# zhangmozhe/Deep-Exemplar-based-Video-Colorization

Measured on AMD Instinct MI355X. Metric: colorized frames/sec/GPU at 216x384; correlation HBM GB/s vs roofline, higher is better.
Workload: dtype f32

## Files before the change

deep-exemplar-based-video-colorization_amd/csrc/conv_mfma.hip:

```cpp
#include "conv_kernel.h"
#include "conv_sk_kernel.h"
#include <algorithm>

#include "conv_wino_kernel.h"

static int virt_dim(int S, int up, int sub) {
    if (up == 2) return S * 2;
    if (sub == 2) return (S + 1) / 2;
    return S;
}

extern "C" int dvc_conv2d_out_hw(const DvcConvDesc* d, int32_t* OH, int32_t* OW) {
    DVC_REQUIRE(d, "dvc_conv2d_out_hw: null descriptor");
    int VH = virt_dim(d->H, d->in_up, d->in_sub), VW = virt_dim(d->W, d->in_up, d->in_sub);
    int ext = d->dil * (d->ksize - 1) + 1;
    *OH = (VH + 2 * d->pad - ext) / d->stride + 1;
    *OW = (VW + 2 * d->pad - ext) / d->stride + 1;
    return 0;
}

static int pick_tw(int OW) {
    int best = 32, best_w = cdiv(OW, 32) * 32;
    for (int tw : {16, 8}) {
        int wpad = cdiv(OW, tw) * tw;
// ... 484 lines not shown
    int m, tr, S;
    wino_plan(d, OH, OW, workspace_bytes > 0, workspace_bytes, &m, &tr, &S);
    DVC_REQUIRE(m >= 0, "dvc_conv2d_winograd_split: no configuration for cfg %d / split_k %d on this layer", d->cfg, d->split_k);
    const int kc = kWinoShapes[m].kc, nch = d->Cin / kc;
    *split = cdiv(nch, cdiv(nch, S));
    *images_per_launch = wino_images_per_launch(d, OH, OW, m, tr, *split, workspace_bytes);
    return 0;
}

static int wino_setup(const DvcConvDesc* d, const DvcConvDesc* d2, const float* x, const float* x2, const float* u_packed,
                      const float* bias, const float* act_slope_ptr, const float* residual, float* y, void* workspace,
                      size_t workspace_bytes, float* pool, long pool_batch_stride, ConvWinoArgs& s, int* m_out, int* tr_out,
                      int* group_out) {
    DVC_REQUIRE(d && x && u_packed && (y || pool), "dvc_conv2d_winograd: null argument");
    DVC_REQUIRE(d->ksize == 3 && d->stride == 1 && (d->dil == 1 || d->dil == 2) && d->pad == d->dil,
                "dvc_conv2d_winograd: needs a 3x3 stride-1 layer with pad == dilation (1 or 2)");
    DVC_REQUIRE(!d->in_prelu, "dvc_conv2d_winograd: no fused input transform on this path");
    DVC_REQUIRE((d->in_up == 1 || d->in_up == 2) && (d->in_sub == 1 || d->in_sub == 2) && !(d->in_up == 2 && d->in_sub == 2),
                "dvc_conv2d_winograd: bad in_up/in_sub");
    DVC_REQUIRE(d->N > 0 && d->Cin > 0 && d->H > 0 && d->W > 0 && d->Cout > 0, "dvc_conv2d_winograd: bad shape");
    DVC_REQUIRE(d->Cin % 8 == 0 && d->Cout % 64 == 0, "dvc_conv2d_winograd: needs Cin %% 8 == 0 and Cout %% 64 == 0 (got %d, %d)",
                d->Cin, d->Cout);
    DVC_REQUIRE((reinterpret_cast<uintptr_t>(u_packed) & 15) == 0, "dvc_conv2d_winograd: weights must be 16-byte aligned");
    DVC_REQUIRE((long)d->Cin * d->H * d->W * 4 < (1L << 31) && (long)d->Cin * 2048 * 4 < (1L << 31),
                "dvc_conv2d_winograd: tensor too large for buffer-descriptor staging");
    s.x2 = nullptr; s.x2_bs = 0; s.cinA = d->Cin; s.H2 = s.W2 = s.VH2 = s.VW2 = 0; s.in_up2 = s.in_sub2 = 1;
    ConvKArgs& a = s.k;
    a.x = x; a.w = u_packed; a.bias = bias; a.in_scale = nullptr; a.in_shift = nullptr;
    a.in_slope_ptr = nullptr; a.act_slope_ptr = act_slope_ptr; a.res = residual; a.y = y;
    a.N = d->N; a.Cin = d->Cin; a.H = d->H; a.W = d->W;
    a.VH = virt_dim(d->H, d->in_up, d->in_sub);
    a.VW = virt_dim(d->W, d->in_up, d->in_sub);
    int32_t OH, OW;
    dvc_conv2d_out_hw(d, &OH, &OW);
    DVC_REQUIRE(OH > 0 && OW > 0, "dvc_conv2d_winograd: empty output");
    if (d->pad_mode == DVC_PAD_REFLECT)
        DVC_REQUIRE(d->pad < a.VH && d->pad < a.VW, "dvc_conv2d_winograd: reflect pad needs pad < input size");
    a.Cout = d->Cout; a.OH = OH; a.OW = OW;
    a.ks = 3; a.stride = 1; a.dil = d->dil; a.pad = d->pad; a.pad_mode = d->pad_mode;
    a.in_up = d->in_up; a.in_sub = d->in_sub; a.act = d->act; a.in_prelu = 0;
    a.act_slope = d->act_slope;
    a.x_bs = d->x_batch_stride ? d->x_batch_stride : (long)d->Cin * d->H * d->W;
    a.y_bs = d->y_batch_stride ? d->y_batch_stride : (long)d->Cout * OH * OW;
    a.res_bs = d->res_batch_stride ? d->res_batch_stride : (long)d->Cout * OH * OW;
    a.cin_pad = d->Cin; a.IH_T = a.IW_T = a.IW_P = 0;
    a.dbg = g_conv_dbg; a.dbg_buf = nullptr; a.w_bs = 0; a.gray = 0;
    s.ss = d->dil;
    const int TY = cdiv(cdiv(OH, s.ss), 2), TX = cdiv(cdiv(OW, s.ss), 2);
    int best_m = -1, best_tr = 1, best_S = 1;
    if (d2) {
        s.x2 = x2;
        s.cinA = d->Cin - d2->Cin;
        s.H2 = d2->H; s.W2 = d2->W;
        s.VH2 = virt_dim(d2->H, d2->in_up, d2->in_sub);
        s.VW2 = virt_dim(d2->W, d2->in_up, d2->in_sub);
        s.in_up2 = d2->in_up; s.in_sub2 = d2->in_sub;
        s.x2_bs = d2->x_batch_stride ? d2->x_batch_stride : (long)d2->Cin * d2->H * d2->W;
        DVC_REQUIRE(s.VH2 == a.VH && s.VW2 == a.VW, "dvc_conv2d_winograd_dual: the two inputs' virtual sizes differ (%d x %d vs %d x %d)",
                    a.VH, a.VW, s.VH2, s.VW2);
        DVC_REQUIRE((long)d2->Cin * d2->H * d2->W * 4 < (1L << 31), "dvc_conv2d_winograd_dual: second input too large");
        a.x_bs = d->x_batch_stride ? d->x_batch_stride : (long)s.cinA * d->H * d->W;
    }
    wino_plan(d, OH, OW, workspace != nullptr, workspace_bytes, &best_m, &best_tr, &best_S, d2 ? 2 : -1);
    DVC_REQUIRE(best_m >= 0, "dvc_conv2d_winograd: no configuration for cfg %d / split_k %d on this layer", d->cfg, d->split_k);
    const int wm = kWinoShapes[best_m].wm, wn = kWinoShapes[best_m].wn, kc = kWinoShapes[best_m].kc;
    const int nch = d->Cin / kc;
    s.blk_y = cdiv(TY, best_tr * wn);
    s.blk_x = cdiv(TX, 32 / best_tr);
    a.chunks_per_split = cdiv(nch, best_S);
    a.split = cdiv(nch, a.chunks_per_split);
    a.part = reinterpret_cast<float*>(workspace);
    s.gx = s.ss * s.ss * s.blk_y * s.blk_x;
    s.gy = d->Cout / (32 * wm);
    const int group = wino_images_per_launch(d, OH, OW, best_m, best_tr, a.split, workspace_bytes);
    DVC_REQUIRE(group >= 0, "dvc_conv2d_winograd: %ld workgroups per image (feature map too large for this path)",
                (long)s.gx * s.gy * a.split);
    DVC_REQUIRE(group > 0, "dvc_conv2d_winograd: split-K workspace too small for one image");
    DVC_REQUIRE(!(d->flags & DVC_CONV_DEFER_REDUCE) || a.split == 1 || group >= d->N,
                "dvc_conv2d_winograd: DVC_CONV_DEFER_REDUCE needs a workspace that holds the partial sums of the whole batch");
    DVC_REQUIRE(!(d->flags & DVC_CONV_DEFER_REDUCE) || a.split == 1 || !residual,
                "dvc_conv2d_winograd: DVC_CONV_DEFER_REDUCE does not carry a residual");
    s.pool_bs = pool_batch_stride ? pool_batch_stride : (long)d->Cout * (OH / 2) * (OW / 2);
    s.pool = pool;
    *m_out = best_m; *tr_out = best_tr; *group_out = group;
    return 0;
}

static dim3 wino_finish_grid(ConvWinoArgs& s, int NB) {
    s.gz = NB * s.k.split;
    s.m_gxy = wino_magic((long)s.gx * s.gy);
    s.m_gx = wino_magic(s.gx);
    s.m_cls = wino_magic((long)s.blk_y * s.blk_x);
    s.m_blkx = wino_magic(s.blk_x);
    s.m_split = wino_magic(s.k.split);
    return dim3((unsigned)(s.gx * s.gy * s.gz));
}

static int wino_reduce(const DvcConvDesc* d, const ConvWinoArgs& s, int NB, int OH, int OW, const float* bias,
                       const float* act_slope_ptr, hipStream_t st) {
    const ConvKArgs& a = s.k;
    const long OHW = (long)OH * OW, per_img = (long)d->Cout * OHW;
    if (a.split > 1 && s.pool) {
        const long windows = (long)d->Cout * ((OH + 1) / 2) * ((OW + 1) / 2);
        hipLaunchKernelGGL(conv_splitk_reduce_pool_kernel, dim3((unsigned)((windows + 255) / 256), NB), dim3(256), 0, st, a.part,
                           a.split, (long)NB * per_img, d->Cout, OH, OW, bias, d->act, d->act_slope, act_slope_ptr, a.y, a.y_bs,
                           s.pool, s.pool_bs);
        DVC_CHECK_LAUNCH("dvc_conv2d_winograd_pool(split-K reduce)");
    } else if (a.split > 1 && !(d->flags & DVC_CONV_DEFER_REDUCE)) {
        const bool v4 = (OHW % 4 == 0) && ((reinterpret_cast<uintptr_t>(a.part) & 15) == 0) && (((long)NB * per_img) % 4 == 0);
        if (v4)
            hipLaunchKernelGGL(conv_splitk_reduce_kernel<4>, dim3((unsigned)((per_img / 4 + 255) / 256), NB), dim3(256), 0, st,
                               a.part, a.split, (long)NB * per_img, d->Cout, OHW, bias, a.res, a.res_bs, d->act,
                               d->act_slope, act_slope_ptr, a.y, a.y_bs);
        else
            hipLaunchKernelGGL(conv_splitk_reduce_kernel<1>, dim3((unsigned)((per_img + 255) / 256), NB), dim3(256), 0, st,
                               a.part, a.split, (long)NB * per_img, d->Cout, OHW, bias, a.res, a.res_bs, d->act,
                               d->act_slope, act_slope_ptr, a.y, a.y_bs);
        DVC_CHECK_LAUNCH("dvc_conv2d_winograd(split-K reduce)");
    }
    return 0;
}

static int wino_run(const DvcConvDesc* d, const DvcConvDesc* d2, const float* x, const float* x2, const float* u_packed,
                    const float* bias, const float* act_slope_ptr, const float* residual, float* y, void* workspace,
                    size_t workspace_bytes, dvcStream stream, float* pool = nullptr, long pool_batch_stride = 0) {
    ConvWinoArgs s;
    int best_m = -1, best_tr = 1, group = 0;
    if (int rc = wino_setup(d, d2, x, x2, u_packed, bias, act_slope_ptr, residual, y, workspace, workspace_bytes, pool,
                            pool_batch_stride, s, &best_m, &best_tr, &group))
        return rc;
    ConvKArgs& a = s.k;
    int32_t OH, OW;
    dvc_conv2d_out_hw(d, &OH, &OW);
    hipStream_t st = (hipStream_t)stream;
    for (int n0 = 0; n0 < d->N; n0 += group) {
        const int NB = std::min(group, d->N - n0);
        a.N = NB;
        a.x = x + (long)n0 * a.x_bs;
        if (d2) s.x2 = x2 + (long)n0 * s.x2_bs;
        a.y = y ? y + (long)n0 * a.y_bs : nullptr;
        s.pool = pool ? pool + (long)n0 * s.pool_bs : nullptr;
        a.res = residual ? residual + (long)n0 * a.res_bs : nullptr;
        DVC_REQUIRE((long)s.gx * s.gy * NB * a.split < (1L << 31), "dvc_conv2d_winograd: grid too large");
        const dim3 grid = wino_finish_grid(s, NB);
        if (d2) conv_wino_launch_m1_dual(best_tr, grid, st, s);
        else if (best_m == 0) conv_wino_launch_m4(best_tr, grid, st, s);
        else if (best_m == 1) conv_wino_launch_m2(best_tr, grid, st, s);
        else if (best_m == 2) conv_wino_launch_m1(best_tr, grid, st, s);
        else conv_wino_launch_m0(best_tr, grid, st, s);
        DVC_CHECK_LAUNCH("dvc_conv2d_winograd");
        if (int rc = wino_reduce(d, s, NB, OH, OW, bias, act_slope_ptr, st)) return rc;
    }
    return 0;
}

extern "C" int dvc_conv2d_winograd_group(const DvcConvGroupItem* items, int32_t n_items, dvcStream stream) {
    DVC_REQUIRE(items && n_items >= 1 && n_items <= WINO_GROUP_MAX, "dvc_conv2d_winograd_group: 1..%d items", WINO_GROUP_MAX);
    hipStream_t st = (hipStream_t)stream;
    ConvWinoGroupArgs g;
    int OHs[WINO_GROUP_MAX], OWs[WINO_GROUP_MAX], order[WINO_GROUP_MAX];
    ConvWinoArgs tmp[WINO_GROUP_MAX];
    int trs[WINO_GROUP_MAX];
    bool together = n_items > 1;
    for (int i = 0; i < n_items; ++i) {
        const DvcConvGroupItem& it = items[i];
        DVC_REQUIRE(it.x && it.u_packed && it.y, "dvc_conv2d_winograd_group: null argument in item %d", i);
// ... 127 lines not shown
```

deep-exemplar-based-video-colorization_amd/csrc/conv_wino_kernel.h:

```cpp
#pragma once
#include <type_traits>

#include "conv_kernel.h"

typedef float f32x4 __attribute__((ext_vector_type(4)));
typedef float f32x2 __attribute__((ext_vector_type(2)));

struct ConvWinoArgs {
    ConvKArgs k;
    int ss;
    int blk_y, blk_x;
    int gx, gy, gz;
    unsigned m_gx, m_gxy, m_cls, m_blkx, m_split;
    const float* x2;
    long x2_bs;
    int cinA, H2, W2, VH2, VW2, in_up2, in_sub2;
    float* pool;
    long pool_bs;
};
__host__ __device__ __forceinline__ unsigned wino_magic(long d) {
    return d > 1 ? (unsigned)(((1ULL << 32) + (unsigned long long)d - 1) / (unsigned long long)d) : 0u;
}
__device__ __forceinline__ int wino_div(int n, unsigned magic) { return magic ? (int)__umulhi((unsigned)n, magic) : n; }

__host__ __device__ constexpr int wino_pitch(int tr) { return tr == 1 ? 66 : tr == 2 ? 48 : tr == 4 ? 24 : 12; }

#define WINO_A10(p) "a" #p "0", "a" #p "1", "a" #p "2", "a" #p "3", "a" #p "4", "a" #p "5", "a" #p "6", "a" #p "7", "a" #p "8", "a" #p "9"
#define WINO_AGPRS                                                                                                     \
    WINO_A10(), WINO_A10(1), WINO_A10(2), WINO_A10(3), WINO_A10(4), WINO_A10(5), WINO_A10(6), WINO_A10(7), WINO_A10(8), \
        WINO_A10(9), WINO_A10(10), WINO_A10(11), "a120", "a121", "a122", "a123", "a124", "a125", "a126", "a127"
#define WINO_MFMA(K, A, B)                                                                \
    asm volatile("s_nop 1\n\tv_mfma_f32_32x32x2_f32 a[%2:%3], %0, %1, a[%2:%3]"            \
                 :                                                                         \
                 : "v"(A), "v"(B), "i"((K) * 16), "i"((K) * 16 + 15)                       \
                 : WINO_AGPRS)
#define WINO_PK_ADD(D, A, B) asm volatile("v_pk_add_f32 %0, %1, %2" : "=v"(D) : "v"(A), "v"(B))
#define WINO_PK_SUB(D, A, B) asm volatile("v_pk_add_f32 %0, %1, %2 neg_lo:[0,1] neg_hi:[0,1]" : "=v"(D) : "v"(A), "v"(B))
#define WINO_PK_MID(D, A, B) \
    asm volatile("v_pk_add_f32 %0, %1, %2 op_sel:[0,1] op_sel_hi:[0,1] neg_hi:[0,1]" : "=v"(D) : "v"(A), "v"(B))

#define WINO_LOADS(D, U, XA, UA, UOFS)                                                                                 \
    asm volatile("ds_read2_b64 %0, %5 offset0:%7 offset1:%8\n\t"                                                        \
                 "ds_read2_b64 %1, %5 offset0:%9 offset1:%10\n\t"                                                       \
                 "ds_read2_b64 %2, %5 offset0:%11 offset1:%12\n\t"                                                      \
                 "ds_read_b128 %3, %6 offset:%13\n\t"                                                                   \
                 "ds_read_b128 %4, %6 offset:%14"                                                                       \
                 : "=&v"(D[0]), "=&v"(D[1]), "=&v"(D[2]), "=&v"(U[0]), "=&v"(U[1])                                      \
                 : "v"(XA), "v"(UA), "i"(0 * (PITCH / 2)), "i"(0 * (PITCH / 2) + 1), "i"(1 * (PITCH / 2)),              \
                   "i"(1 * (PITCH / 2) + 1), "i"(2 * (PITCH / 2)), "i"(2 * (PITCH / 2) + 1), "i"((UOFS) + 0),           \
                   "i"((UOFS) + 512)                                                                                    \
                 : "memory")
#define WINO_WAIT_LOADS(D, U)                                                                 \
    asm volatile("s_waitcnt lgkmcnt(0)"                                                        \
                 : "+v"(D[0]), "+v"(D[1]), "+v"(D[2]), "+v"(U[0]), "+v"(U[1])                  \
                 :                                                                             \
                 : "memory")

#define WINO_S_ADD(D, A, B) asm volatile("v_add_f32 %0, %1, %2" : "=v"(D) : "v"(A), "v"(B))
#define WINO_S_SUB(D, A, B) asm volatile("v_sub_f32 %0, %1, %2" : "=v"(D) : "v"(A), "v"(B))

__device__ __forceinline__ int wino_stored_offset(int VH, int VW, int W, int in_up, int in_sub, int pad_mode, int vy, int vx) {
    int sy = map_virtual(vy, VH, pad_mode);
    int sx = map_virtual(vx, VW, pad_mode);
    if (sy < 0 || sx < 0) return -1;
    if (in_up == 2) {
        sy >>= 1;
        sx >>= 1;
    } else if (in_sub == 2) {
        sy <<= 1;
        sx <<= 1;
    }
    return sy * W + sx;
}

#define WINO_NBUF 3
__host__ __device__ constexpr int wino_xs_floats(int wm, int wn, int tr, int kc) {
    return ((kc * (2 * tr * wn + 2) * wino_pitch(tr) + 128 * wm * wn - 1) / (128 * wm * wn)) * (128 * wm * wn);
}
__host__ __device__ constexpr int wino_us_floats(int wm, int kc) { return wm * kc * 128 * 4; }

template <int WM, int WN, int TR, int KC, int VAR = 0, bool DUAL = false, class SA = ConvWinoArgs>
__device__ __forceinline__ void conv_wino_body(const SA& s, const int wlog, float* const xsb, float* const usb) {
#if defined(__HIP_DEVICE_COMPILE__)
    const auto& a = s.k;
    constexpr int NPAIR = WM * WN;
    constexpr int NT = 128 * NPAIR;
    constexpr int TC = 32 / TR;
    constexpr int PR = 2 * TR * WN + 2;
    constexpr int PC = 2 * TC + 2;
    constexpr int PITCH = wino_pitch(TR);
    constexpr int plane = PR * PITCH;
    constexpr int EPT = (KC * plane + NT - 1) / NT;
    constexpr int C_XS = EPT * NT;
    static_assert(C_XS == wino_xs_floats(WM, WN, TR, KC), "LDS size helper out of step");
    constexpr int UQ = WM * KC * 128;
    static_assert(UQ * 4 == wino_us_floats(WM, KC), "LDS size helper out of step");
    static_assert(UQ % NT == 0, "whole staging instructions");
    static_assert(PITCH >= PC && PITCH % 2 == 0 && plane % 2 == 0 && KC % 4 == 0, "aligned patch rows, even K-steps per chunk");
    static_assert(2 * (PITCH / 2) + 1 < 256, "ds_read2_b64 offsets are 8 bits");
    constexpr int WPT = UQ / NT;
    constexpr int NI = EPT + WPT;
    static_assert(2 * NI < 64, "vmcnt is 6 bits");
    constexpr int KS = KC / 2;
    constexpr int NBUF = WINO_NBUF;
    constexpr int OOB = (int)0x80000000;
    static_assert(NBUF * UQ * 4 >= 2 * NPAIR * 32 * 64, "the output exchange fits in the filter buffers");

    const int tid = threadIdx.x;
    const int lane = tid & 63, wave = __builtin_amdgcn_readfirstlane(tid >> 6);
    const int l31 = lane & 31, hi = lane >> 5;
    const int ph = wave / NPAIR, pair = wave % NPAIR;
    const int wm = pair / WN, wn = pair % WN;
    const int tr = l31 / TC, tc = l31 % TC;
    const int ss = s.ss;
    const int bz = wino_div(wlog, s.m_gxy), r_xy = wlog - bz * (s.gx * s.gy);
    const int by = wino_div(r_xy, s.m_gx), bx = r_xy - by * s.gx;
    const int per_cls = s.blk_y * s.blk_x;
    const int cls = wino_div(bx, s.m_cls), brem = bx - cls * per_cls;
    const int py = ss == 2 ? cls >> 1 : 0, px = ss == 2 ? cls & 1 : 0;
    const int tyb = wino_div(brem, s.m_blkx);
    const int ty0 = tyb * (TR * WN), tx0 = (brem - tyb * s.blk_x) * TC;
    const int b0 = by * WM;
    const int n = wino_div(bz, s.m_split), ksplit = bz - n * a.split;
    const int HWi = a.H * a.W;

    const int nchunks_all = a.Cin / KC;
    const int c_begin = ksplit * a.chunks_per_split;
    const int c_end = min(nchunks_all, c_begin + a.chunks_per_split);

    int gofs[EPT], wrel[WPT];
#pragma unroll
    for (int i = 0; i < WPT; ++i) {
        const int q = tid + i * NT;
        wrel[i] = ((q / (KC * 128)) * a.Cin * 128 + q % (KC * 128)) * 16;
    }
    __amdgpu_buffer_rsrc_t rs_w =
        __builtin_amdgcn_make_buffer_rsrc((void*)(a.w + (long)b0 * a.Cin * 512), 0, WM * a.Cin * 2048, 0x00020000);
    auto issue_w = [&](int c, int buf) {
        const int sw = c * KC * 2048;
        float* us = usb + buf * (UQ * 4);
#pragma unroll
        for (int i = 0; i < WPT; ++i)
            __builtin_amdgcn_raw_ptr_buffer_load_lds(rs_w, (CONV_AS3 void*)(us + (i * NT + wave * 64) * 4), 16, wrel[i], sw, 0, 0);
    };
    issue_w(c_begin, 0);
    asm volatile(".set wino_i, 0\n\t.rept 128\n\tv_accvgpr_write_b32 a[wino_i], 0\n\t.set wino_i, wino_i + 1\n\t.endr" ::: WINO_AGPRS);
#pragma unroll
    for (int t = 0; t < EPT; ++t) {
        const int e = tid + t * NT;
        const int c = e / plane, rem = e - c * plane;
        const int iy = rem / PITCH, ix = rem - iy * PITCH;
        int g = -1;
        if (e < KC * plane && ix < PC) {
            const int o = stored_offset(a, ss * (2 * ty0 - 1 + iy) + py, ss * (2 * tx0 - 1 + ix) + px);
            if (o >= 0) g = c * HWi + o;
        }
        gofs[t] = g >= 0 ? g * 4 : OOB;
    }
    const int cinA = DUAL ? s.cinA : a.Cin;
    __amdgpu_buffer_rsrc_t rs_x =
        __builtin_amdgcn_make_buffer_rsrc((void*)(a.x + (long)n * a.x_bs), 0, cinA * HWi * 4, 0x00020000);
    int gofs2[DUAL ? EPT : 1];
    const int HWi2 = DUAL ? s.H2 * s.W2 : 0;
    if (DUAL) {
#pragma unroll
        for (int t = 0; t < EPT; ++t) {
            const int e = tid + t * NT;
            const int c = e / plane, rem = e - c * plane;
            const int iy = rem / PITCH, ix = rem - iy * PITCH;
            int g = -1;
            if (e < KC * plane && ix < PC) {
                const int o = wino_stored_offset(s.VH2, s.VW2, s.W2, s.in_up2, s.in_sub2, a.pad_mode, ss * (2 * ty0 - 1 + iy) + py,
                                                 ss * (2 * tx0 - 1 + ix) + px);
                if (o >= 0) g = c * HWi2 + o;
            }
            gofs2[DUAL ? t : 0] = g >= 0 ? g * 4 : OOB;
        }
    }
    __amdgpu_buffer_rsrc_t rs_x2 = rs_x;
    if (DUAL)
        rs_x2 = __builtin_amdgcn_make_buffer_rsrc((void*)(s.x2 + (long)n * s.x2_bs), 0, (a.Cin - cinA) * HWi2 * 4, 0x00020000);
    const int nchA = cinA / KC;
    auto issue_x = [&](int c, int buf) {
        float* xs = xsb + buf * C_XS;
        const bool first = !DUAL || c < nchA;
        const __amdgpu_buffer_rsrc_t rs = first ? rs_x : rs_x2;
        const int sx = first ? c * KC * HWi * 4 : (c - nchA) * KC * HWi2 * 4;
#pragma unroll
        for (int t = 0; t < EPT; ++t) {
            const int go = first ? gofs[t] : gofs2[DUAL ? t : 0];
            __builtin_amdgcn_raw_ptr_buffer_load_lds(rs, (CONV_AS3 void*)(xs + t * NT + wave * 64), 4, go, sx, 0, 0);
        }
    };
    auto issue = [&](int c, int buf) {
        issue_x(c, buf);
        issue_w(c, buf);
    };

    const unsigned xlane =
        (unsigned)(size_t)(CONV_AS3 float*)xsb + (hi * plane + (2 * (wn * TR + tr) + ph) * PITCH + 2 * tc) * 4;
    const unsigned ulane = (unsigned)(size_t)(CONV_AS3 float*)usb + (((wm * KC + hi) * 4 + 2 * ph) * 32 + l31) * 16;

    constexpr bool BRANCH_FREE = VAR != 3;
    issue_x(c_begin, 0);
    if (BRANCH_FREE) {
        issue(min(c_begin + 1, c_end - 1), 1);
        issue(min(c_begin + 2, c_end - 1), 2);
        asm volatile("s_waitcnt vmcnt(%0)" ::"n"(2 * NI) : "memory");
    } else {
        if (c_begin + 1 < c_end) issue(c_begin + 1, 1);
        if (c_begin + 2 < c_end) issue(c_begin + 2, 2);
        if (c_begin + 2 < c_end) asm volatile("s_waitcnt vmcnt(%0)" ::"n"(2 * NI) : "memory");
        else if (c_begin + 1 < c_end) asm volatile("s_waitcnt vmcnt(%0)" ::"n"(NI) : "memory");
        else asm volatile("s_waitcnt vmcnt(0)" ::: "memory");
    }
    __builtin_amdgcn_s_barrier();

    const float slope = a.act_slope_ptr ? *a.act_slope_ptr : a.act_slope;
    const long OHW = (long)a.OH * a.OW;
    const bool partial = a.split > 1;
    float* yb = partial ? a.part + ((long)ksplit * a.N + n) * a.Cout * OHW : a.y + (long)n * a.y_bs;
    const float* rb = (!partial && a.res) ? a.res + (long)n * a.res_bs : nullptr;

    auto run = [&](auto PHC) {
        constexpr int PH = decltype(PHC)::value;
        f32x4 D[2][3], U[2][2];
        f32x2 V03[2][2], V12[2][2];
        auto lo = [](const f32x4& v) { return __builtin_shufflevector(v, v, 0, 1); };
        auto hh = [](const f32x4& v) { return __builtin_shufflevector(v, v, 2, 3); };
        auto transform_a = [&](const f32x4 (&d)[3], f32x2 (&tl)[2], f32x2 (&th)[2]) {
            if (VAR == 1) {
                if (PH == 0) {
                    WINO_S_SUB(tl[0].x, d[0].x, d[2].x); WINO_S_SUB(tl[0].y, d[0].y, d[2].y);
                    WINO_S_SUB(th[0].x, d[0].z, d[2].z); WINO_S_SUB(th[0].y, d[0].w, d[2].w);
                    WINO_S_ADD(tl[1].x, d[1].x, d[2].x); WINO_S_ADD(tl[1].y, d[1].y, d[2].y);
                    WINO_S_ADD(th[1].x, d[1].z, d[2].z); WINO_S_ADD(th[1].y, d[1].w, d[2].w);
                } else {
                    WINO_S_SUB(tl[0].x, d[1].x, d[0].x); WINO_S_SUB(tl[0].y, d[1].y, d[0].y);
                    WINO_S_SUB(th[0].x, d[1].z, d[0].z); WINO_S_SUB(th[0].y, d[1].w, d[0].w);
                    WINO_S_SUB(tl[1].x, d[0].x, d[2].x); WINO_S_SUB(tl[1].y, d[0].y, d[2].y);
                    WINO_S_SUB(th[1].x, d[0].z, d[2].z); WINO_S_SUB(th[1].y, d[0].w, d[2].w);
                }
                return;
            }
            if (PH == 0) {
                WINO_PK_SUB(tl[0], lo(d[0]), lo(d[2]));
                WINO_PK_SUB(th[0], hh(d[0]), hh(d[2]));
                WINO_PK_ADD(tl[1], lo(d[1]), lo(d[2]));
                WINO_PK_ADD(th[1], hh(d[1]), hh(d[2]));
            } else {
                WINO_PK_SUB(tl[0], lo(d[1]), lo(d[0]));
                WINO_PK_SUB(th[0], hh(d[1]), hh(d[0]));
                WINO_PK_SUB(tl[1], lo(d[0]), lo(d[2]));
                WINO_PK_SUB(th[1], hh(d[0]), hh(d[2]));
            }
        };
        auto transform_b = [&](const f32x2& tl, const f32x2& th, f32x2& v03, f32x2& v12) {
            if (VAR == 1) {
                WINO_S_SUB(v03.x, tl.x, th.x); WINO_S_SUB(v03.y, tl.y, th.y);
                WINO_S_ADD(v12.x, th.x, tl.y); WINO_S_SUB(v12.y, th.x, tl.y);
                return;
            }
            WINO_PK_SUB(v03, tl, th);
            WINO_PK_MID(v12, th, tl);
        };
        {
            f32x2 tl[2], th[2];
            WINO_LOADS(D[0], U[0], xlane, ulane, 0);
            WINO_WAIT_LOADS(D[0], U[0]);
            transform_a(D[0], tl, th);
            transform_b(tl[0], th[0], V03[0][0], V12[0][0]);
            transform_b(tl[1], th[1], V03[0][1], V12[0][1]);
        }

        int buf = 0;
        for (int c = c_begin; c < c_end; ++c) {
            const unsigned xb = xlane + buf * (C_XS * 4), ub = ulane + buf * (UQ * 16);
            const int nbuf = buf == NBUF - 1 ? 0 : buf + 1;
            const unsigned xbn = xlane + nbuf * (C_XS * 4), ubn = ulane + nbuf * (UQ * 16);
            const bool more = c + 1 < c_end;
#pragma unroll
            for (int ks = 0; ks < KS; ++ks) {
                const int cs = ks & 1, ns = cs ^ 1;
                const bool last = ks == KS - 1;
                f32x2 tl[2], th[2];
                WINO_MFMA(0, U[cs][0].x, V03[cs][0].x);
                if (!last) {
                    WINO_LOADS(D[ns], U[ns], xb + (ks + 1) * (2 * plane * 4), ub, (ks + 1) * 4096);
                } else if (BRANCH_FREE) {
                    asm volatile("s_waitcnt vmcnt(%0)" ::"n"(NI) : "memory");
                    __builtin_amdgcn_s_barrier();
                    issue(min(c + 3, c_end - 1), buf);
                    WINO_LOADS(D[ns], U[ns], xbn, ubn, 0);
                } else if (more) {
                    if (c + 2 < c_end) asm volatile("s_waitcnt vmcnt(%0)" ::"n"(NI) : "memory");
                    else asm volatile("s_waitcnt vmcnt(0)" ::: "memory");
                    __builtin_amdgcn_s_barrier();
                    if (c + 3 < c_end) issue(c + 3, buf);
                    WINO_LOADS(D[ns], U[ns], xbn, ubn, 0);
                }
                __builtin_amdgcn_sched_barrier(0);
                WINO_MFMA(1, U[cs][0].y, V12[cs][0].x);
                WINO_MFMA(2, U[cs][0].z, V12[cs][0].y);
                WINO_MFMA(3, U[cs][0].w, V03[cs][0].y);
                WINO_WAIT_LOADS(D[ns], U[ns]);
                __builtin_amdgcn_sched_barrier(0);
                transform_a(D[ns], tl, th);
                __builtin_amdgcn_sched_barrier(0);
                WINO_MFMA(4, U[cs][1].x, V03[cs][1].x);
                transform_b(tl[0], th[0], V03[ns][0], V12[ns][0]);
                __builtin_amdgcn_sched_barrier(0);
                WINO_MFMA(5, U[cs][1].y, V12[cs][1].x);
                transform_b(tl[1], th[1], V03[ns][1], V12[ns][1]);
                __builtin_amdgcn_sched_barrier(0);
                WINO_MFMA(6, U[cs][1].z, V12[cs][1].y);
                WINO_MFMA(7, U[cs][1].w, V03[cs][1].y);
                __builtin_amdgcn_sched_barrier(0);
            }
            buf = nbuf;
        }
        asm volatile("s_waitcnt vmcnt(0)" ::: "memory");
        __builtin_amdgcn_s_barrier();

        float* ex = usb;
        asm volatile("s_nop 15\n\ts_nop 7" ::: WINO_AGPRS);
        auto partial_out = [&](auto RC, float (&o)[4]) {
            constexpr int r = decltype(RC)::value;
            float m[8];
#pragma unroll
            for (int k = 0; k < 8; ++k) asm volatile("v_accvgpr_read_b32 %0, a[%1]" : "=v"(m[k]) : "i"(k * 16 + r) : WINO_AGPRS);
            float s0[4], s1[4];
#pragma unroll
            for (int j = 0; j < 4; ++j) {
                if (PH == 0) {
                    s0[j] = m[j] + m[4 + j];
                    s1[j] = m[4 + j];
                } else {
                    s0[j] = m[j];
                    s1[j] = -m[j] - m[4 + j];
                }
            }
            o[0] = s0[0] + s0[1] + s0[2];
            o[1] = s0[1] - s0[2] - s0[3];
            o[2] = s1[0] + s1[1] + s1[2];
            o[3] = s1[1] - s1[2] - s1[3];
        };
        auto for8 = [&](auto f) {
            f(std::integral_constant<int, 0>{}); f(std::integral_constant<int, 1>{}); f(std::integral_constant<int, 2>{});
            f(std::integral_constant<int, 3>{}); f(std::integral_constant<int, 4>{}); f(std::integral_constant<int, 5>{});
            f(std::integral_constant<int, 6>{}); f(std::integral_constant<int, 7>{});
        };
        {
            float* mine = ex + (wave * 32) * 64 + lane;
            for8([&](auto IC) {
                constexpr int i = decltype(IC)::value;
                float o[4];
                partial_out(std::integral_constant<int, 8 * (1 - PH) + i>{}, o);
#pragma unroll
                for (int q = 0; q < 4; ++q) mine[(i * 4 + q) * 64] = o[q];
            });
        }
        __syncthreads();
        const float* theirs = ex + ((PH == 0 ? wave + NPAIR : wave - NPAIR) * 32) * 64 + lane;
        const int u0 = 2 * (ty0 + wn * TR + tr), x0 = 2 * (tx0 + tc);
        const int oy0 = ss * u0 + py, oy1 = ss * (u0 + 1) + py;
        const int ox0 = ss * x0 + px, ox1 = ss * (x0 + 1) + px;
        const bool okx0 = ox0 < a.OW, okx1 = ox1 < a.OW;
        const bool pairst = ss == 1 && okx1 && (a.OW & 1) == 0;
        const bool pool_here = !partial && s.pool;
        float* pb = pool_here ? s.pool + (long)n * s.pool_bs : nullptr;
        const long PHW = (long)(a.OH >> 1) * (a.OW >> 1);
        for8([&](auto IC) {
            constexpr int i = decltype(IC)::value;
            constexpr int r = 8 * PH + i;
            float o[4];
            partial_out(std::integral_constant<int, r>{}, o);
#pragma unroll
            for (int q = 0; q < 4; ++q) {
                const float t = theirs[(i * 4 + q) * 64];
                o[q] = PH == 0 ? o[q] + t : t + o[q];
            }
            const int co = (b0 + wm) * 32 + (r & 3) + 8 * (r >> 2) + 4 * hi;
            const float bias = (!partial && a.bias) ? a.bias[co] : 0.f;
            float pooled = 0.f;
#pragma unroll
            for (int p = 0; p < 2; ++p) {
                const int oy = p ? oy1 : oy0;
                if (oy >= a.OH) continue;
                const long row = (long)co * OHW + (long)oy * a.OW;
                float v0 = o[2 * p] + bias, v1 = o[2 * p + 1] + bias;
                if (rb) {
                    if (okx0) v0 += rb[row + ox0];
                    if (okx1) v1 += rb[row + ox1];
                }
                if (!partial) {
                    v0 = apply_act(v0, a.act, slope);
                    v1 = apply_act(v1, a.act, slope);
                }
                if (pool_here) {
                    const float m = fmaxf(v0, v1);
                    pooled = p ? fmaxf(pooled, m) : m;
                    if (p && okx1) pb[(long)co * PHW + (long)(oy0 >> 1) * (a.OW >> 1) + (ox0 >> 1)] = pooled;
                    if (!a.y) continue;
                }
                if (pairst && VAR == 2) {
                    union { float2 f; unsigned long long u; } cv;
                    cv.f = make_float2(v0, v1);
                    __hip_atomic_store(reinterpret_cast<unsigned long long*>(yb + row + ox0), cv.u, __ATOMIC_RELAXED, __HIP_MEMORY_SCOPE_AGENT);
                } else if (pairst) {
                    *reinterpret_cast<float2*>(yb + row + ox0) = make_float2(v0, v1);
                } else {
                    if (okx0) yb[row + ox0] = v0;
                    if (okx1) yb[row + ox1] = v1;
                }
            }
        });
    };
    if (ph) run(std::integral_constant<int, 1>{});
    else run(std::integral_constant<int, 0>{});
#endif
}

template <int WM, int WN, int TR, int KC, int VAR = 0, bool DUAL = false>
__global__ __launch_bounds__(128 * WM * WN) __attribute__((amdgpu_waves_per_eu(2, 2))) void conv_wino_kernel(ConvWinoArgs s) {
    __shared__ __attribute__((aligned(16))) float xsb[WINO_NBUF * wino_xs_floats(WM, WN, TR, KC)];
    __shared__ __attribute__((aligned(16))) float usb[WINO_NBUF * wino_us_floats(WM, KC)];
    const int G = s.gx * s.gy * s.gz;
    const int xq = G / 8, xr = G % 8, xcd = blockIdx.x % 8, xi = blockIdx.x / 8;
    const int wlog = (xcd < xr ? xcd * (xq + 1) : xr * (xq + 1) + (xcd - xr) * xq) + xi;
    conv_wino_body<WM, WN, TR, KC, VAR, DUAL>(s, wlog, xsb, usb);
}

#define WINO_GROUP_MAX 4
struct ConvWinoGroupArgs {
    ConvWinoArgs item[WINO_GROUP_MAX];
    int per_xcd[WINO_GROUP_MAX + 1];
    int tr[WINO_GROUP_MAX];
    int n;
};
typedef __attribute__((address_space(4))) ConvWinoArgs ConvWinoArgsK;
template <int WM, int WN, int KC>
__global__ __launch_bounds__(128 * WM * WN) __attribute__((amdgpu_waves_per_eu(2, 2))) void conv_wino_group_kernel(ConvWinoGroupArgs g) {
    constexpr int XS = wino_xs_floats(WM, WN, 1, KC) > wino_xs_floats(WM, WN, 8, KC) ? wino_xs_floats(WM, WN, 1, KC) : wino_xs_floats(WM, WN, 8, KC);
    static_assert(XS >= wino_xs_floats(WM, WN, 2, KC) && XS >= wino_xs_floats(WM, WN, 4, KC), "largest patch buffer");
#if defined(__HIP_DEVICE_COMPILE__)
    __shared__ __attribute__((aligned(16))) float xsb[WINO_NBUF * XS];
// ... 83 lines not shown
```

deep-exemplar-based-video-colorization_amd/dvc_amd/ops.py:

```python
import ctypes
import os as _os
import sys
from typing import NamedTuple

import torch

from . import _lib
from ._lib import DvcConvDesc, DvcConvGroupItem, DvcInstNormItem

ACT_NONE, ACT_RELU, ACT_PRELU, ACT_LEAKY, ACT_TANH128 = 0, 1, 2, 3, 4
PAD_ZERO, PAD_REFLECT = 0, 1
EPS64 = sys.float_info.epsilon


def _p(t):
    return None if t is None else ctypes.c_void_p(t.data_ptr())


def _pv(t):
    return None if t is None else t.data_ptr()


_raw_stream = getattr(torch._C, "_cuda_getCurrentRawStream", None)
_raw_device = getattr(torch._C, "_cuda_getDevice", None)
# ... 29 lines not shown

def _need_all(**named):
    for name, t in named.items():
        _need(t, name)


_ws_cache = {}
_ws_scope = None


class workspace_scope:

    def __init__(self, store):
        self.store = store

    def __enter__(self):
        global _ws_scope
        self.prev, _ws_scope = _ws_scope, self.store
        return self.store

    def __exit__(self, *exc):
        global _ws_scope
        _ws_scope = self.prev


def _workspace(device, nbytes, tag="corr"):
    if _ws_scope is not None:
        cache, key = _ws_scope, (tag, device.index)
    else:
        cache, key = _ws_cache, (tag, device.index, _stream_handle())
    ws = cache.get(key)
    if ws is None or ws.numel() < nbytes:
        ws = torch.empty(nbytes, device=device, dtype=torch.uint8)
        cache[key] = ws
    return ws


conv_record = None
layer_record = None


def _on_unless_0(v):
    return v != "0"


def _on_if_1(v):
    return v == "1"


def _memo_mode(v):
    return {"0": "off", "verify": "verify"}.get(v, "on")


def _layer_names(v):
    return None if v is None else frozenset(v.split(","))


class _Switch(NamedTuple):
    getter: str
    setter: str
    var: str
    env: str
    default: str
    parse: object
    launch: bool


_SWITCHES = (
    _Switch("autotune_enabled", None, "_autotune", "DVC_AUTOTUNE", "0", _on_if_1, True),
    _Switch("ws_conv_enabled", "set_ws_conv", "_ws_conv", "DVC_WS_CONV", "1", _on_unless_0, True),
    _Switch("pool_fusion", "set_pool_fusion", "_pool_fusion", "DVC_POOL_FUSION", "1", _on_unless_0, True),
    _Switch("dual_conv_enabled", "set_dual_conv", "_dual_conv", "DVC_DUAL_CONV", "1", _on_if_1, True),
    _Switch("fuse_reduce", "set_fuse_reduce", "_fuse_reduce", "DVC_FUSE_REDUCE", "1", _on_if_1, True),
    _Switch("conv_algo", None, "_conv_algo", "DVC_CONV_ALGO", "auto", str, True),
    _Switch("exemplar_memo_mode", None, "_exemplar_memo", "DVC_EXEMPLAR_MEMO", "1", _memo_mode, False),
    _Switch("gemm_lib", "set_gemm_lib", "_gemm_lib", "DVC_GEMM_LIB", "1", _on_unless_0, False),
    _Switch("gray_fusion", "set_gray_fusion", "_gray_fusion", "DVC_GRAY_FUSION", "1", _on_unless_0, True),
    _Switch("group_heads", "set_group_heads", "_group_heads", "DVC_GROUP_HEADS", "1", _on_unless_0, True),
    _Switch("fold_merge", "set_fold_merge", "_fold_merge", "DVC_FOLD_MERGE", "1", _on_if_1, True),
    _Switch("batch_plan_enabled", None, "_batch_plan", None, "0", _on_if_1, True),
    _Switch("direct_layers", None, "DEFAULT_DIRECT_LAYERS", "DVC_DIRECT_LAYERS", None, _layer_names, True),
)


def _flag_functions(var, getter, setter):
    g = globals()

    def get():
        return g[var]

    def set_(flag=True):
        g[var] = bool(flag)
    get.__name__ = get.__qualname__ = getter
    set_.__name__ = set_.__qualname__ = setter
    return get, set_


for _sw in _SWITCHES:
    globals()[_sw.var] = _sw.parse(_os.environ.get(_sw.env, _sw.default) if _sw.env else _sw.default)
    if _sw.setter:
        globals()[_sw.getter], globals()[_sw.setter] = _flag_functions(_sw.var, _sw.getter, _sw.setter)
del _sw


def launch_epoch():
    g = globals()
    return tuple(g[sw.getter]() for sw in _SWITCHES if sw.launch)


def autotune_enabled():
    return _autotune


def set_autotune(flag=True):
    global _autotune
    _autotune = bool(flag)
    if _autotune:
        _load_tuned()


def conv_algo():
    return _conv_algo


def set_conv_algo(algo):
    global _conv_algo
    if algo not in ("auto", "speed", "direct", "winograd"):
        raise ValueError("conv algo must be 'auto', 'speed', 'direct' or 'winograd'")
    _conv_algo = algo


def exemplar_memo_enabled():
    return _exemplar_memo != "off"


def exemplar_memo_mode():
    return _exemplar_memo


def set_exemplar_memo(flag=True):
    global _exemplar_memo
    _exemplar_memo = "verify" if flag == "verify" else ("on" if flag else "off")


_direct_layers = None


def direct_layers():
    if _direct_layers is not None:
        return _direct_layers
    if DEFAULT_DIRECT_LAYERS is not None:
        return DEFAULT_DIRECT_LAYERS
    from . import arch
    return arch.DIRECT_LAYERS


def set_direct_layers(names=None):
    global _direct_layers
    _direct_layers = None if names is None else frozenset(names)


DEFER_REDUCE = 1
BATCH_PLAN = 2
GRAY_INPUT = 4


class batch_plan:

    def __init__(self, on=True):
        self.on = bool(on)

    def __enter__(self):
        global _batch_plan
        self.prev, _batch_plan = _batch_plan, self.on
        return self

    def __exit__(self, *exc):
        global _batch_plan
        _batch_plan = self.prev


def batch_plan_enabled():
    return _batch_plan


def _plan_flags(N):
    return BATCH_PLAN if (_batch_plan and N > 1) else 0


_tuned = {}

_cache_path = _os.environ.get("DVC_AUTOTUNE_CACHE")
_cache_loaded = False


def _load_tuned():
    global _cache_loaded
    if _cache_loaded or not _cache_path:
        return
    _cache_loaded = True
    try:
        import json
        with open(_cache_path) as f:
            for k, v in json.load(f).items():
                _tuned[tuple(json.loads(k))] = tuple(v)
    except (OSError, ValueError):
        pass


def _save_tuned():
    if not _cache_path:
        return
    import json
    tmp = _cache_path + ".tmp%d" % _os.getpid()
    with open(tmp, "w") as f:
        json.dump({json.dumps(list(k)): list(v) for k, v in _tuned.items()}, f)
    _os.replace(tmp, _cache_path)


def autotune_table():
    return dict(_tuned)


if _autotune:
    _load_tuned()


_TUNE_SPLITS = tuple(int(v) for v in _os.environ.get("DVC_TUNE_SPLITS", "1,2,3,4,6,8").split(","))
_TUNE_STREAMK = tuple((int(a), int(b)) for a, b in (v.split(":") for v in _os.environ.get("DVC_TUNE_STREAMK", "36:2,36:1").split(",") if v))


def _tune_conv(lib, d, tensors):
    x, w_packed, bias, in_scale, in_shift, in_slope_t, act_slope_t, residual, out = tensors
    if residual is not None and residual.data_ptr() == out.data_ptr():
        out = torch.empty_like(out)
    ws = _workspace(x.device, CONV_WORKSPACE_BYTES, "conv")
    stream = _stream()

    def launch():
        return lib.dvc_conv2d(ctypes.byref(d), _p(x), _p(w_packed), _p(bias), _p(in_scale), _p(in_shift),
                              _p(in_slope_t), _p(act_slope_t), _p(residual), _p(out),
                              ctypes.c_void_p(ws.data_ptr()), ws.numel(), stream)

    best, best_t = (-1, 0), float("inf")
    e0, e1 = torch.cuda.Event(enable_timing=True), torch.cuda.Event(enable_timing=True)

    def time_it():
        launch()
        e0.record()
        for _ in range(3):
            launch()
        e1.record()
        e1.synchronize()
        return e0.elapsed_time(e1)

    d.cfg, d.split_k = -1, 0
    if launch() == 0:
        best, best_t = (-1, 0), time_it()
    for cfg in (0, 1, 2, 3, 4):
        for sk in _TUNE_SPLITS:
            d.cfg, d.split_k = cfg, sk
            if launch() != 0:
                break
            t = time_it()
            if t < best_t:
                best, best_t = (cfg, sk), t
    for cfg, per_cu in _TUNE_STREAMK:
        d.cfg, d.split_k = cfg, per_cu
        if launch() != 0:
            continue
# ... 954 lines not shown
```

include/dvc_hip.h:

```cpp
#ifndef DVC_HIP_H
#define DVC_HIP_H

#include <stddef.h>
#include <stdint.h>

#ifdef __cplusplus
extern "C" {
#endif

#pragma GCC visibility push(default)

typedef void* dvcStream;

#define DVC_ABI_VERSION 20

int dvc_abi_version(void);
const char* dvc_last_error(void);

enum { DVC_ACT_NONE = 0, DVC_ACT_RELU = 1, DVC_ACT_PRELU = 2, DVC_ACT_LEAKY = 3, DVC_ACT_TANH128 = 4 };
enum { DVC_PAD_ZERO = 0, DVC_PAD_REFLECT = 1 };

typedef struct DvcConvDesc {
    int32_t N, Cin, H, W;
    int32_t Cout;
    int32_t ksize;
    int32_t stride;
    int32_t dil;
    int32_t pad;
    int32_t pad_mode;
    int32_t in_up;
    int32_t in_sub;
    int32_t act;
    float   act_slope;
    int32_t in_prelu;
    int32_t cfg;
    int32_t split_k;
    int64_t x_batch_stride;
    int64_t y_batch_stride;
    int64_t res_batch_stride;
    int32_t flags;
    int64_t w_batch_stride;
} DvcConvDesc;
#define DVC_CONV_DEFER_REDUCE 1
#define DVC_CONV_BATCH_PLAN 2
#define DVC_CONV_GRAY_INPUT 4

int dvc_conv2d_out_hw(const DvcConvDesc* d, int32_t* OH, int32_t* OW);

int dvc_conv2d(const DvcConvDesc* d,
               const float* x, const float* w_packed, const float* bias ,
               const float* in_scale , const float* in_shift ,
               const float* in_slope_ptr ,
               const float* act_slope_ptr ,
               const float* residual , float* y,
               void* workspace , size_t workspace_bytes,
               dvcStream stream);

size_t dvc_winograd_weight_floats(int32_t Cout, int32_t Cin);
int dvc_winograd_pack_weight(const float* w, int32_t Cout, int32_t Cin, float* u_packed, dvcStream stream);
int dvc_conv2d_winograd_split(const DvcConvDesc* d, size_t workspace_bytes, int32_t* split, int32_t* images_per_launch);
int dvc_conv2d_winograd(const DvcConvDesc* d, const float* x, const float* u_packed,
                        const float* bias , const float* act_slope_ptr ,
                        const float* residual , float* y,
                        void* workspace , size_t workspace_bytes, dvcStream stream);
int dvc_conv2d_winograd_pool(const DvcConvDesc* d, const float* x, const float* u_packed, const float* bias ,
                             const float* act_slope_ptr , float* y , float* y_pool,
                             int64_t pool_batch_stride, void* workspace , size_t workspace_bytes, dvcStream stream);
int dvc_conv2d_winograd_dual(const DvcConvDesc* dA, const DvcConvDesc* dB, const float* xA, const float* xB,
                             const float* u_packed_cat, const float* bias ,
                             const float* act_slope_ptr , float* y,
                             void* workspace , size_t workspace_bytes, dvcStream stream);

int dvc_conv2d_ws_eligible(const DvcConvDesc* d);
int dvc_conv2d_ws_pack_weight(const float* w, int32_t Cout, int32_t Cin, float* u_packed, dvcStream stream);
int dvc_conv2d_ws(const DvcConvDesc* d, const float* x, const float* u_packed, const float* bias ,
                  const float* act_slope_ptr , float* y, dvcStream stream);

typedef struct DvcConvGroupItem {
    DvcConvDesc d;
    const float* x;
    const float* u_packed;
    const float* bias;
    const float* act_slope_ptr;
    const float* residual;
    float* y;
    void* workspace;
    size_t workspace_bytes;
} DvcConvGroupItem;
int dvc_conv2d_winograd_group(const DvcConvGroupItem* items, int32_t n_items, dvcStream stream);

int dvc_conv1x1_small(const float* x, const float* w, const float* bias, int32_t N, int32_t Cin,
                      int32_t HW, int32_t Cout, int32_t act, float* y, dvcStream stream);

int dvc_instnorm_stats(const float* x, int32_t N, int32_t C, int32_t HW, int64_t x_batch_stride,
                       float eps, const float* chan_scale, float* scale, float* shift,
                       dvcStream stream);

int dvc_affine_act(const float* x, const float* scale, const float* shift, const float* residual,
                   const float* slope_ptr, int32_t N, int32_t C, int32_t H, int32_t W, int32_t up,
                   int32_t rpad, int64_t x_batch_stride, int64_t res_batch_stride,
                   int64_t y_batch_stride, float* y, dvcStream stream);

int dvc_instnorm_apply(const float* x, const float* residual , const float* slope_ptr ,
                       const float* chan_scale , float eps, int32_t N, int32_t C, int32_t H,
                       int32_t W, int32_t up, int32_t sub, int32_t rpad, int64_t x_batch_stride,
                       int64_t res_batch_stride, int64_t y_batch_stride, float* y,
                       float* scale_out, float* shift_out,
                       const float* chan_scale2 , int32_t sub2, float* y2 ,
                       dvcStream stream);
int dvc_instnorm_apply_partials(const float* part, int32_t S, const float* bias, int32_t act, float act_slope,
                                const float* act_slope_ptr, const float* residual, const float* slope_ptr,
                                const float* chan_scale, float eps, int32_t N, int32_t C, int32_t H, int32_t W, int32_t up,
                                int32_t sub, int32_t rpad, int64_t res_batch_stride, int64_t y_batch_stride, float* y,
                                float* scale_out, float* shift_out, const float* chan_scale2, int32_t sub2, float* y2,
                                dvcStream stream);

typedef struct DvcInstNormItem {
    const float* x;
    int32_t S;
    const float* bias;
    int32_t act;
    float act_slope;
    const float* act_slope_ptr;
    const float* residual;
    const float* slope_ptr;
    const float* chan_scale;
    float eps;
    int32_t N, C, H, W, up, sub, rpad;
// ... 135 lines not shown
```

Measured before the change: 432.6.

## Skip zero Winograd input-transform terms for nearest-upsampled inputs

```diff
diff --git a/deep-exemplar-based-video-colorization_amd/csrc/conv_mfma.hip b/deep-exemplar-based-video-colorization_amd/csrc/conv_mfma.hip
--- a/deep-exemplar-based-video-colorization_amd/csrc/conv_mfma.hip
+++ b/deep-exemplar-based-video-colorization_amd/csrc/conv_mfma.hip
@@ -590,6 +590,12 @@
                 "dvc_conv2d_winograd: DVC_CONV_DEFER_REDUCE does not carry a residual");
     s.pool_bs = pool_batch_stride ? pool_batch_stride : (long)d->Cout * (OH / 2) * (OW / 2);
     s.pool = pool;
+    s.up_sparse = 0;
+    if (!(d->flags & DVC_CONV_UP_DENSE) && s.ss == 1 && a.VH % 2 == 0 && a.VW % 2 == 0) {
+        if (d->in_up == 2 && d->in_sub == 1) s.up_sparse |= 1;
+        if (d2 && d2->in_up == 2 && d2->in_sub == 1) s.up_sparse |= 2;
+        if (s.up_sparse && !(kDvcDebug && (g_conv_dbg & 16384))) s.up_sparse |= 4;
+    }
     *m_out = best_m; *tr_out = best_tr; *group_out = group;
     return 0;
 }
diff --git a/deep-exemplar-based-video-colorization_amd/csrc/conv_wino_kernel.h b/deep-exemplar-based-video-colorization_amd/csrc/conv_wino_kernel.h
--- a/deep-exemplar-based-video-colorization_amd/csrc/conv_wino_kernel.h
+++ b/deep-exemplar-based-video-colorization_amd/csrc/conv_wino_kernel.h
@@ -17,6 +17,7 @@
     int cinA, H2, W2, VH2, VW2, in_up2, in_sub2;
     float* pool;
     long pool_bs;
+    int up_sparse;
 };
 __host__ __device__ __forceinline__ unsigned wino_magic(long d) {
     return d > 1 ? (unsigned)(((1ULL << 32) + (unsigned long long)d - 1) / (unsigned long long)d) : 0u;
@@ -55,6 +56,17 @@
                  : "+v"(D[0]), "+v"(D[1]), "+v"(D[2]), "+v"(U[0]), "+v"(U[1])                  \
                  :                                                                             \
                  : "memory")
+
+#define WINO_LOADS_UP1(D, U, XA, UA, UOFS)                                                                             \
+    asm volatile("ds_read2_b64 %0, %3 offset0:%5 offset1:%6\n\t"                                                        \
+                 "ds_read2_b64 %1, %3 offset0:%7 offset1:%8\n\t"                                                        \
+                 "ds_read_b128 %2, %4 offset:%9"                                                                        \
+                 : "=&v"(D[0]), "=&v"(D[2]), "=&v"(U[1])                                                                \
+                 : "v"(XA), "v"(UA), "i"(0 * (PITCH / 2)), "i"(0 * (PITCH / 2) + 1), "i"(2 * (PITCH / 2)),              \
+                   "i"(2 * (PITCH / 2) + 1), "i"((UOFS) + 512)                                                          \
+                 : "memory")
+#define WINO_WAIT_LOADS_UP1(D, U) \
+    asm volatile("s_waitcnt lgkmcnt(0)" : "+v"(D[0]), "+v"(D[2]), "+v"(U[1]) : : "memory")
 
 #define WINO_S_ADD(D, A, B) asm volatile("v_add_f32 %0, %1, %2" : "=v"(D) : "v"(A), "v"(B))
 #define WINO_S_SUB(D, A, B) asm volatile("v_sub_f32 %0, %1, %2" : "=v"(D) : "v"(A), "v"(B))
@@ -109,7 +121,9 @@
     const int tid = threadIdx.x;
     const int lane = tid & 63, wave = __builtin_amdgcn_readfirstlane(tid >> 6);
     const int l31 = lane & 31, hi = lane >> 5;
-    const int ph = wave / NPAIR, pair = wave % NPAIR;
+    const int usp = s.up_sparse;
+    const int flip = (usp & 4) ? (wlog & 1) : 0;
+    const int ph = (wave / NPAIR) ^ flip, pair = wave % NPAIR;
     const int wm = pair / WN, wn = pair % WN;
     const int tr = l31 / TC, tc = l31 % TC;
     const int ss = s.ss;
@@ -228,7 +242,12 @@
         f32x2 V03[2][2], V12[2][2];
         auto lo = [](const f32x4& v) { return __builtin_shufflevector(v, v, 0, 1); };
         auto hh = [](const f32x4& v) { return __builtin_shufflevector(v, v, 2, 3); };
-        auto transform_a = [&](const f32x4 (&d)[3], f32x2 (&tl)[2], f32x2 (&th)[2]) {
+        auto transform_a = [&](const f32x4 (&d)[3], f32x2 (&tl)[2], f32x2 (&th)[2], bool up1 = false) {
+            if (up1) {
+                WINO_PK_SUB(tl[1], lo(d[0]), lo(d[2]));
+                WINO_PK_SUB(th[1], hh(d[0]), hh(d[2]));
+                return;
+            }
             if (VAR == 1) {
                 if (PH == 0) {
                     WINO_S_SUB(tl[0].x, d[0].x, d[2].x); WINO_S_SUB(tl[0].y, d[0].y, d[2].y);
@@ -274,50 +293,86 @@
         }
 
         int buf = 0;
-        for (int c = c_begin; c < c_end; ++c) {
-            const unsigned xb = xlane + buf * (C_XS * 4), ub = ulane + buf * (UQ * 16);
-            const int nbuf = buf == NBUF - 1 ? 0 : buf + 1;
-            const unsigned xbn = xlane + nbuf * (C_XS * 4), ubn = ulane + nbuf * (UQ * 16);
-            const bool more = c + 1 < c_end;
-#pragma unroll
-            for (int ks = 0; ks < KS; ++ks) {
-                const int cs = ks & 1, ns = cs ^ 1;
-                const bool last = ks == KS - 1;
-                f32x2 tl[2], th[2];
-                WINO_MFMA(0, U[cs][0].x, V03[cs][0].x);
-                if (!last) {
-                    WINO_LOADS(D[ns], U[ns], xb + (ks + 1) * (2 * plane * 4), ub, (ks + 1) * 4096);
-                } else if (BRANCH_FREE) {
-                    asm volatile("s_waitcnt vmcnt(%0)" ::"n"(NI) : "memory");
-                    __builtin_amdgcn_s_barrier();
-                    issue(min(c + 3, c_end - 1), buf);
-                    WINO_LOADS(D[ns], U[ns], xbn, ubn, 0);
-                } else if (more) {
-                    if (c + 2 < c_end) asm volatile("s_waitcnt vmcnt(%0)" ::"n"(NI) : "memory");
-                    else asm volatile("s_waitcnt vmcnt(0)" ::: "memory");
-                    __builtin_amdgcn_s_barrier();
-                    if (c + 3 < c_end) issue(c + 3, buf);
-                    WINO_LOADS(D[ns], U[ns], xbn, ubn, 0);
-                }
-                __builtin_amdgcn_sched_barrier(0);
-                WINO_MFMA(1, U[cs][0].y, V12[cs][0].x);
-                WINO_MFMA(2, U[cs][0].z, V12[cs][0].y);
-                WINO_MFMA(3, U[cs][0].w, V03[cs][0].y);
-                WINO_WAIT_LOADS(D[ns], U[ns]);
-                __builtin_amdgcn_sched_barrier(0);
-                transform_a(D[ns], tl, th);
-                __builtin_amdgcn_sched_barrier(0);
-                WINO_MFMA(4, U[cs][1].x, V03[cs][1].x);
-                transform_b(tl[0], th[0], V03[ns][0], V12[ns][0]);
-                __builtin_amdgcn_sched_barrier(0);
-                WINO_MFMA(5, U[cs][1].y, V12[cs][1].x);
-                transform_b(tl[1], th[1], V03[ns][1], V12[ns][1]);
-                __builtin_amdgcn_sched_barrier(0);
-                WINO_MFMA(6, U[cs][1].z, V12[cs][1].y);
-                WINO_MFMA(7, U[cs][1].w, V03[cs][1].y);
-                __builtin_amdgcn_sched_barrier(0);
-            }
-            buf = nbuf;
+        auto chunks = [&](auto SPC, auto PREFC, const int c0, const int c1) __attribute__((always_inline)) {
+            constexpr bool SP = decltype(SPC)::value, PREF = decltype(PREFC)::value;
+            constexpr bool UP1 = SP && PH == 1;
+            for (int c = c0; c < c1; ++c) {
+                const unsigned xb = xlane + buf * (C_XS * 4), ub = ulane + buf * (UQ * 16);
+                const int nbuf = buf == NBUF - 1 ? 0 : buf + 1;
+                const unsigned xbn = xlane + nbuf * (C_XS * 4), ubn = ulane + nbuf * (UQ * 16);
+                const bool more = c + 1 < c_end;
+#pragma unroll
+                for (int ks = 0; ks < KS; ++ks) {
+                    const int cs = ks & 1, ns = cs ^ 1;
+                    const bool last = ks == KS - 1;
+                    const bool nup1 = (last ? PREF : SP) && PH == 1;
+                    f32x2 tl[2], th[2];
+                    if (UP1) WINO_MFMA(4, U[cs][1].x, V03[cs][1].x);
+                    else WINO_MFMA(0, U[cs][0].x, V03[cs][0].x);
+                    if (!last) {
+                        if (nup1) WINO_LOADS_UP1(D[ns], U[ns], xb + (ks + 1) * (2 * plane * 4), ub, (ks + 1) * 4096);
+                        else WINO_LOADS(D[ns], U[ns], xb + (ks + 1) * (2 * plane * 4), ub, (ks + 1) * 4096);
+                    } else if (BRANCH_FREE) {
+                        asm volatile("s_waitcnt vmcnt(%0)" ::"n"(NI) : "memory");
+                        __builtin_amdgcn_s_barrier();
+                        issue(min(c + 3, c_end - 1), buf);
+                        if (nup1) WINO_LOADS_UP1(D[ns], U[ns], xbn, ubn, 0);
+                        else WINO_LOADS(D[ns], U[ns], xbn, ubn, 0);
+                    } else if (more) {
+                        if (c + 2 < c_end) asm volatile("s_waitcnt vmcnt(%0)" ::"n"(NI) : "memory");
+                        else asm volatile("s_waitcnt vmcnt(0)" ::: "memory");
+                        __builtin_amdgcn_s_barrier();
+                        if (c + 3 < c_end) issue(c + 3, buf);
+                        if (nup1) WINO_LOADS_UP1(D[ns], U[ns], xbn, ubn, 0);
+                        else WINO_LOADS(D[ns], U[ns], xbn, ubn, 0);
+                    }
+                    __builtin_amdgcn_sched_barrier(0);
+                    if (UP1) {
+                        WINO_MFMA(5, U[cs][1].y, V12[cs][1].x);
+                    } else {
+                        WINO_MFMA(1, U[cs][0].y, V12[cs][0].x);
+                        if (!SP) WINO_MFMA(2, U[cs][0].z, V12[cs][0].y);
+                        WINO_MFMA(3, U[cs][0].w, V03[cs][0].y);
+                    }
+                    if (nup1) WINO_WAIT_LOADS_UP1(D[ns], U[ns]);
+                    else WINO_WAIT_LOADS(D[ns], U[ns]);
+                    __builtin_amdgcn_sched_barrier(0);
+                    transform_a(D[ns], tl, th, nup1);
+                    __builtin_amdgcn_sched_barrier(0);
+                    if (!UP1) WINO_MFMA(4, U[cs][1].x, V03[cs][1].x);
+                    if (!nup1) transform_b(tl[0], th[0], V03[ns][0], V12[ns][0]);
+                    __builtin_amdgcn_sched_barrier(0);
+                    if (UP1) WINO_MFMA(7, U[cs][1].w, V03[cs][1].y);
+                    else WINO_MFMA(5, U[cs][1].y, V12[cs][1].x);
+                    transform_b(tl[1], th[1], V03[ns][1], V12[ns][1]);
+                    __builtin_amdgcn_sched_barrier(0);
+                    if (!UP1) {
+                        if (!SP) WINO_MFMA(6, U[cs][1].z, V12[cs][1].y);
+                        WINO_MFMA(7, U[cs][1].w, V03[cs][1].y);
+                        __builtin_amdgcn_sched_barrier(0);
+                    }
+                }
+                buf = nbuf;
+            }
+        };
+        auto input_run = [&](const bool sparse, auto FOLLOWS, const int c0, const int c1) __attribute__((always_inline)) {
+            constexpr std::false_type dense_c{};
+            constexpr std::true_type sparse_c{};
+            if (!sparse) {
+                chunks(dense_c, dense_c, c0, c1);
+            } else if (!decltype(FOLLOWS)::value) {
+                chunks(sparse_c, sparse_c, c0, c1);
+            } else {
+                chunks(sparse_c, sparse_c, c0, c1 - 1);
+                if (c0 < c1) chunks(sparse_c, dense_c, c1 - 1, c1);
+            }
+        };
+        if (DUAL) {
+            const int c_mid = min(max(nchA, c_begin), c_end);
+            input_run((usp & 1) != 0, std::true_type{}, c_begin, c_mid);
+            input_run((usp & 2) != 0, std::false_type{}, c_mid, c_end);
+        } else {
+            input_run((usp & 1) != 0, std::false_type{}, c_begin, c_end);
         }
         asm volatile("s_waitcnt vmcnt(0)" ::: "memory");
         __builtin_amdgcn_s_barrier();
@@ -361,7 +416,7 @@
             });
         }
         __syncthreads();
-        const float* theirs = ex + ((PH == 0 ? wave + NPAIR : wave - NPAIR) * 32) * 64 + lane;
+        const float* theirs = ex + ((wave < NPAIR ? wave + NPAIR : wave - NPAIR) * 32) * 64 + lane;
         const int u0 = 2 * (ty0 + wn * TR + tr), x0 = 2 * (tx0 + tc);
         const int oy0 = ss * u0 + py, oy1 = ss * (u0 + 1) + py;
         const int ox0 = ss * x0 + px, ox1 = ss * (x0 + 1) + px;
diff --git a/deep-exemplar-based-video-colorization_amd/dvc_amd/ops.py b/deep-exemplar-based-video-colorization_amd/dvc_amd/ops.py
--- a/deep-exemplar-based-video-colorization_amd/dvc_amd/ops.py
+++ b/deep-exemplar-based-video-colorization_amd/dvc_amd/ops.py
@@ -135,6 +135,11 @@
     _Switch("direct_layers", None, "DEFAULT_DIRECT_LAYERS", "DVC_DIRECT_LAYERS", None, _layer_names, True),
 )
 
+_VARIANT_SWITCHES = (
+    _Switch("wino_up_sparse", "set_wino_up_sparse", "_wino_up_sparse", "DVC_WINO_UP_SPARSE", "1", _on_unless_0, False),
+)
+
+
 
 def _flag_functions(var, getter, setter):
     g = globals()
@@ -149,7 +154,7 @@
     return get, set_
 
 
-for _sw in _SWITCHES:
+for _sw in _SWITCHES + _VARIANT_SWITCHES:
     globals()[_sw.var] = _sw.parse(_os.environ.get(_sw.env, _sw.default) if _sw.env else _sw.default)
     if _sw.setter:
         globals()[_sw.getter], globals()[_sw.setter] = _flag_functions(_sw.var, _sw.getter, _sw.setter)
@@ -216,6 +221,7 @@
 DEFER_REDUCE = 1
 BATCH_PLAN = 2
 GRAY_INPUT = 4
+UP_DENSE = 8
 
 
 class batch_plan:
@@ -238,7 +244,7 @@
 
 
 def _plan_flags(N):
-    return BATCH_PLAN if (_batch_plan and N > 1) else 0
+    return (BATCH_PLAN if (_batch_plan and N > 1) else 0) | (0 if _wino_up_sparse else UP_DENSE)
 
 
 _tuned = {}
diff --git a/include/dvc_hip.h b/include/dvc_hip.h
--- a/include/dvc_hip.h
+++ b/include/dvc_hip.h
@@ -44,6 +44,7 @@
 #define DVC_CONV_DEFER_REDUCE 1
 #define DVC_CONV_BATCH_PLAN 2
 #define DVC_CONV_GRAY_INPUT 4
+#define DVC_CONV_UP_DENSE 8
 
 int dvc_conv2d_out_hw(const DvcConvDesc* d, int32_t* OH, int32_t* OW);
 
```

Result: no change. 436.6 (median of 6 runs) (+0.9%).
